# mmsyan/GoPairingBasedCryptography

Measured on AMD Instinct MI355X. Metric: BN254 pairings/s at batch 2^20 per GPU (+ G1/G2 scalar-mults/s at the same batch in roofline.scalar_mul), higher is better.
Workload: dtype int64; 1 GPU; configs[1]: batch of 1048576 independent bn254.Pair on random (G1,G2) points per GPU; batch_per_gpu=1048576

## Files before the change

gopairingbasedcryptography_amd/csrc/curve29.hip.hpp:

```cpp
#ifndef GPBC_CURVE29_HIP_HPP
#define GPBC_CURVE29_HIP_HPP
#include "tower29.hip.hpp"

namespace gpbc {

GPBC_INLINE Fe g_add(const Fe &a, const Fe &b) { return fe_add(a, b); }
GPBC_INLINE Fe g_sub(const Fe &a, const Fe &b) { return fe_sub(a, b); }
GPBC_INLINE Fe g_dbl(const Fe &a) { return fe_dbl(a); }
GPBC_INLINE Fe g_norm(const Fe &a) { return fe_norm(a); }
GPBC_INLINE Fe g_mul8n(const Fe &a) { return fe_mul8_norm(a); }
GPBC_INLINE Fe g_mul(const Fe &a, const Fe &b) { return fe_mul(a, b); }
GPBC_INLINE Fe g_sqr(const Fe &a) { return fe_sqr(a); }
GPBC_INLINE Fe g_inv(const Fe &a) { return fe_inv(a); }
GPBC_INLINE bool g_is_zero(const Fe &a) { return fe_is_zero(a); }
GPBC_INLINE void g_set_one(Fe &a) { a = fe_one(); }
GPBC_INLINE void g_set_zero(Fe &a) { a = fe_zero(); }
GPBC_INLINE F2 g_add(const F2 &a, const F2 &b) { return f2_add(a, b); }
GPBC_INLINE F2 g_sub(const F2 &a, const F2 &b) { return f2_sub(a, b); }
GPBC_INLINE F2 g_dbl(const F2 &a) { return f2_dbl(a); }
GPBC_INLINE F2 g_norm(const F2 &a) { return f2_norm(a); }
GPBC_INLINE F2 g_mul8n(const F2 &a) { return f2_mul8_norm(a); }
GPBC_INLINE F2 g_mul(const F2 &a, const F2 &b) { return f2_mul(a, b); }
GPBC_INLINE F2 g_sqr(const F2 &a) { return f2_sqr(a); }
GPBC_INLINE F2 g_inv(const F2 &a) { return f2_inv(a); }
// ... 48 lines not shown
    F Z1Z1 = g_sqr(p.z), Z2Z2 = g_sqr(q.z);
    F U1 = g_mul(p.x, Z2Z2), U2 = g_mul(q.x, Z1Z1);
    F S1 = g_mul(g_mul(p.y, q.z), Z2Z2), S2 = g_mul(g_mul(q.y, p.z), Z1Z1);
    F H = g_sub(U2, U1);
    F rr = g_sub(S2, S1);
    if (g_is_zero(H)) {
        if (g_is_zero(rr)) { jac_dbl(r, p); return; }
        jac_set_inf(r);
        return;
    }
    rr = g_norm(g_dbl(rr));
    F HH = g_sqr(H);
    F I = g_norm(g_dbl(g_dbl(HH)));
    F J = g_mul(H, I);
    F V = g_mul(U1, I);
    F x3 = g_norm(g_sub(g_sub(g_sqr(rr), J), g_dbl(V)));
    F y3 = g_norm(g_sub(g_mul(rr, g_sub(V, x3)), g_dbl(g_mul(S1, J))));
    F z3 = g_mul(g_norm(g_sub(g_sub(g_sqr(g_norm(g_add(p.z, q.z))), Z1Z1), Z2Z2)), H);
    r.x = x3; r.y = y3; r.z = z3; r.inf = false;
}
template <class F> GPBC_INLINE void jac_to_affine(AffP<F> &r, const JacP<F> &p) {
    if (p.inf) { g_set_zero(r.x); g_set_zero(r.y); r.inf = true; return; }
    F zi = g_inv(p.z);
    F zi2 = g_sqr(zi);
    r.x = g_mul(p.x, zi2);
    r.y = g_mul(p.y, g_mul(zi2, zi));
    r.inf = false;
}

struct GlvSplit { uint32_t k1[5], k2[5]; bool neg1, neg2; };

template <int NA, int NB, int NO> GPBC_INLINE void mp_mul(uint32_t (&out)[NO], const uint32_t (&a)[NA], const uint32_t (&b)[NB]) {
    uint64_t carry = 0;
#pragma unroll
    for (int k = 0; k < NO; k++) {
        uint64_t lo = carry, hi = 0;
#pragma unroll
        for (int i = 0; i < NA; i++) {
            const int j = k - i;
            if (j < 0 || j >= NB) continue;
            uint64_t p = (uint64_t)a[i] * (uint64_t)b[j];
            lo += p & 0xffffffffu;
            hi += p >> 32;
        }
        out[k] = (uint32_t)lo;
        carry = (lo >> 32) + hi;
    }
}
template <int N> GPBC_INLINE void mp_sub(uint32_t (&r)[N], const uint32_t (&a)[N], const uint32_t (&b)[N]) {
    uint64_t borrow = 0;
#pragma unroll
    for (int i = 0; i < N; i++) {
        uint64_t d = (uint64_t)a[i] - b[i] - borrow;
        r[i] = (uint32_t)d;
        borrow = (d >> 32) & 1;
    }
}
GPBC_INLINE void glv_split(GlvSplit &o, const uint32_t kin[8]) {
    constexpr uint32_t R32[8] = GLV_R32, G1[3] = GLV_G1, G2[5] = GLV_G2, A1[2] = GLV_A1, A2[4] = GLV_A2, B1[4] = GLV_B1ABS, B2[2] = GLV_B2;
    uint32_t k[8];
#pragma unroll
    for (int i = 0; i < 8; i++) k[i] = kin[i];
    for (int rep = 0; rep < 6; rep++) {
        uint32_t d[8];
        uint64_t borrow = 0;
#pragma unroll
        for (int i = 0; i < 8; i++) { uint64_t t = (uint64_t)k[i] - R32[i] - borrow; d[i] = (uint32_t)t; borrow = (t >> 32) & 1; }
#pragma unroll
        for (int i = 0; i < 8; i++) k[i] = borrow ? k[i] : d[i];
    }
    uint32_t p1[11], p2[13];
    mp_mul<8, 3, 11>(p1, k, G1);
    mp_mul<8, 5, 13>(p2, k, G2);
    uint32_t c1[3] = {p1[8], p1[9], p1[10]}, c2[5] = {p2[8], p2[9], p2[10], p2[11], p2[12]};
    uint32_t t1[5], t2[5], t3[5], t4[5], k5[5] = {k[0], k[1], k[2], k[3], k[4]}, r1[5], r2[5];
    mp_mul<3, 2, 5>(t1, c1, A1);
    mp_mul<5, 4, 5>(t2, c2, A2);
    mp_sub<5>(r1, k5, t1);
    mp_sub<5>(r1, r1, t2);
    mp_mul<3, 4, 5>(t3, c1, B1);
    mp_mul<5, 2, 5>(t4, c2, B2);
    mp_sub<5>(r2, t3, t4);
    o.neg1 = (r1[4] >> 31) != 0;
    o.neg2 = (r2[4] >> 31) != 0;
    uint32_t zero[5] = {0, 0, 0, 0, 0}, n1[5], n2[5];
    mp_sub<5>(n1, zero, r1);
    mp_sub<5>(n2, zero, r2);
#pragma unroll
    for (int i = 0; i < 5; i++) { o.k1[i] = o.neg1 ? n1[i] : r1[i]; o.k2[i] = o.neg2 ? n2[i] : r2[i]; }
}

GPBC_INLINE Fe glv_phi_x(const Fe &x) { constexpr int32_t B[NL] = GLV_BETA_G1; return fe_mul(x, fe_const(B)); }
GPBC_INLINE F2 glv_phi_x(const F2 &x) { constexpr int32_t B[NL] = GLV_BETA_G2; return f2_mul_fe(x, fe_const(B)); }
GPBC_INLINE Fe g_neg(const Fe &a) { return fe_neg(a); }
GPBC_INLINE F2 g_neg(const F2 &a) { return f2_neg(a); }

template <class F> GPBC_INLINE F g_sel(bool c, const F &a, const F &b);
template <> GPBC_INLINE Fe g_sel<Fe>(bool c, const Fe &a, const Fe &b) {
    Fe r;
#pragma unroll
    for (int i = 0; i < NL; i++) r.v[i] = c ? a.v[i] : b.v[i];
#ifdef GPBC_BOUNDS
    for (int i = 0; i < NL; i++) { r.lo[i] = a.lo[i] < b.lo[i] ? a.lo[i] : b.lo[i]; r.hi[i] = a.hi[i] > b.hi[i] ? a.hi[i] : b.hi[i]; }
    r.vb = a.vb > b.vb ? a.vb : b.vb;
#endif
    return r;
}
template <> GPBC_INLINE F2 g_sel<F2>(bool c, const F2 &a, const F2 &b) { return F2{g_sel<Fe>(c, a.a0, b.a0), g_sel<Fe>(c, a.a1, b.a1)}; }

template <class F> GPBC_INLINE JacP<F> jac_phi(const JacP<F> &p, bool flip) {
    return JacP<F>{glv_phi_x(p.x), flip ? g_neg(p.y) : p.y, p.z, p.inf};
}
struct alignas(16) TabQuad { int32_t a, b, c, d; };
template <class F> struct TabLayout;
template <> struct TabLayout<Fe> { static constexpr int ENTRY_DWORDS = 32; };
template <> struct TabLayout<F2> { static constexpr int ENTRY_DWORDS = 64; };
template <class F> constexpr int glv_table_dwords() { return 16 * TabLayout<F>::ENTRY_DWORDS; }
GPBC_INLINE void tab_put(TabQuad *q, const Fe &x, const Fe &y) {
    q[0] = TabQuad{x.v[0], x.v[1], x.v[2], x.v[3]};
    q[1] = TabQuad{x.v[4], x.v[5], x.v[6], x.v[7]};
    q[2] = TabQuad{x.v[8], y.v[0], y.v[1], y.v[2]};
    q[3] = TabQuad{y.v[3], y.v[4], y.v[5], y.v[6]};
    q[4] = TabQuad{y.v[7], y.v[8], 0, 0};
}
GPBC_INLINE void tab_get(const TabQuad *q, Fe &x, Fe &y) {
    TabQuad t0 = q[0], t1 = q[1], t2 = q[2], t3 = q[3], t4 = q[4];
    x.v[0] = t0.a; x.v[1] = t0.b; x.v[2] = t0.c; x.v[3] = t0.d; x.v[4] = t1.a; x.v[5] = t1.b; x.v[6] = t1.c; x.v[7] = t1.d; x.v[8] = t2.a;
    y.v[0] = t2.b; y.v[1] = t2.c; y.v[2] = t2.d; y.v[3] = t3.a; y.v[4] = t3.b; y.v[5] = t3.c; y.v[6] = t3.d; y.v[7] = t4.a; y.v[8] = t4.b;
    GPBC_B(set_class_n(x, 1.5); set_class_n(y, 1.5);)
}
GPBC_INLINE void tab_store(int32_t *mem, int idx, const AffP<Fe> &p) { tab_put(reinterpret_cast<TabQuad *>(mem + idx * 32), p.x, p.y); }
GPBC_INLINE void tab_store(int32_t *mem, int idx, const AffP<F2> &p) {
    TabQuad *q = reinterpret_cast<TabQuad *>(mem + idx * 64);
    tab_put(q, p.x.a0, p.x.a1);
    tab_put(q + 5, p.y.a0, p.y.a1);
}
GPBC_INLINE void tab_load(const int32_t *mem, int idx, AffP<Fe> &p) { tab_get(reinterpret_cast<const TabQuad *>(mem + idx * 32), p.x, p.y); p.inf = false; }
GPBC_INLINE void tab_load(const int32_t *mem, int idx, AffP<F2> &p) {
    const TabQuad *q = reinterpret_cast<const TabQuad *>(mem + idx * 64);
    tab_get(q, p.x.a0, p.x.a1);
    tab_get(q + 5, p.y.a0, p.y.a1);
    p.inf = false;
}
template <class F> GPBC_NOINLINE void glv_table29(int32_t *tab, F &W, const AffP<F> &p1, const AffP<F> &p2, bool flip) {
    F one;
    g_set_one(one);
    JacP<F> J[11];
    JacP<F> p1j{p1.x, p1.y, one, false};
    jac_dbl(J[0], p1j);
    jac_add_mixed(J[1], J[0], p1);
    jac_add_mixed(J[2], p1j, p2);
    jac_dbl(J[3], J[2]);
    jac_add(J[4], J[3], J[2]);
    JacP<F> d2 = jac_phi(J[0], flip), t2 = jac_phi(J[1], flip);
    jac_add_mixed(J[5], d2, p1);
    jac_add_mixed(J[6], J[0], p2);
    jac_add_mixed(J[7], t2, p1);
    jac_add_mixed(J[8], J[1], p2);
    jac_add_mixed(J[9], J[7], p1);
    jac_add_mixed(J[10], J[8], p2);
    F pre[11], l[11];
    F run = one;
    for (int i = 0; i < 11; i++) { pre[i] = run; run = g_mul(run, J[i].z); }
    W = run;
    run = one;
    for (int i = 10; i >= 0; i--) { l[i] = g_mul(pre[i], run); run = g_mul(run, J[i].z); }
    static constexpr int IDX[11] = {8, 12, 5, 10, 15, 6, 9, 7, 13, 11, 14};
    F l2d = one, l3d = one, l2t = one, l3t = one;
    for (int i = 0; i < 11; i++) {
        F l2 = g_sqr(l[i]), l3 = g_mul(l2, l[i]);
        tab_store(tab, IDX[i], AffP<F>{g_mul(J[i].x, l2), g_mul(J[i].y, l3), false});
        if (i == 0) { l2d = l2; l3d = l3; }
        if (i == 1) { l2t = l2; l3t = l3; }
    }
    tab_store(tab, 2, AffP<F>{g_mul(d2.x, l2d), g_mul(d2.y, l3d), false});
    tab_store(tab, 3, AffP<F>{g_mul(t2.x, l2t), g_mul(t2.y, l3t), false});
    F w2 = g_sqr(W), w3 = g_mul(w2, W);
    tab_store(tab, 4, AffP<F>{g_mul(p1.x, w2), g_mul(p1.y, w3), false});
    tab_store(tab, 1, AffP<F>{g_mul(p2.x, w2), g_mul(p2.y, w3), false});
}
template <class F> GPBC_INLINE void scalar_mul29_jac(JacP<F> &acc, const AffP<F> &base, const uint32_t k[8], int32_t *tab) {
    GlvSplit s;
    glv_split(s, k);
    jac_set_inf(acc);
    int top = 159;
    while (top >= 0 && !(((s.k1[top >> 5] | s.k2[top >> 5]) >> (top & 31)) & 1)) top--;
    if (base.inf || top < 0) return;
    AffP<F> p1{base.x, s.neg1 ? g_neg(base.y) : base.y, false};
    AffP<F> p2{glv_phi_x(base.x), s.neg2 ? g_neg(base.y) : base.y, false};
    F W;
    glv_table29<F>(tab, W, p1, p2, s.neg1 != s.neg2);
    for (int i = top >> 1; i >= 0; i--) {
        const int b = 2 * i;
        const int idx = 4 * (int)((s.k1[b >> 5] >> (b & 31)) & 3) + (int)((s.k2[b >> 5] >> (b & 31)) & 3);
        AffP<F> t;
        tab_load(tab, idx, t);
        jac_dbl(acc, acc);
        jac_dbl(acc, acc);
        if (idx) jac_add_mixed(acc, acc, t);
    }
    if (!acc.inf) acc.z = g_mul(acc.z, W);
}
struct GlsSplit { uint32_t k[4][3]; bool neg[4]; };
GPBC_INLINE void gls_split(GlsSplit &o, const uint32_t kin[8]) {
    constexpr uint32_t R32[8] = GLV_R32, G[4][7] = GLS_G, BM[4][4][3] = GLS_BMAG;
    constexpr int GN[4] = GLS_GNEG, BN[4][4] = GLS_BNEG;
    uint32_t k[8];
#pragma unroll
    for (int i = 0; i < 8; i++) k[i] = kin[i];
    for (int rep = 0; rep < 6; rep++) {
        uint32_t d[8];
        uint64_t borrow = 0;
#pragma unroll
        for (int i = 0; i < 8; i++) { uint64_t t = (uint64_t)k[i] - R32[i] - borrow; d[i] = (uint32_t)t; borrow = (t >> 32) & 1; }
#pragma unroll
        for (int i = 0; i < 8; i++) k[i] = borrow ? k[i] : d[i];
    }
    uint32_t c[4][3];
#pragma unroll
    for (int j = 0; j < 4; j++) {
        uint32_t p[11];
        mp_mul<8, 7, 11>(p, k, G[j]);
        c[j][0] = p[8]; c[j][1] = p[9]; c[j][2] = p[10];
    }
#pragma unroll
    for (int i = 0; i < 4; i++) {
        uint32_t acc[3] = {i == 0 ? k[0] : 0u, i == 0 ? k[1] : 0u, i == 0 ? k[2] : 0u};
#pragma unroll
        for (int j = 0; j < 4; j++) {
            uint32_t t[3], r[3];
            mp_mul<3, 3, 3>(t, c[j], BM[j][i]);
            const bool plus = (GN[j] != 0) != (BN[j][i] != 0);
            if (plus) {
                uint64_t cy = 0;
#pragma unroll
                for (int w = 0; w < 3; w++) { uint64_t v = (uint64_t)acc[w] + t[w] + cy; r[w] = (uint32_t)v; cy = v >> 32; }
            } else mp_sub<3>(r, acc, t);
            acc[0] = r[0]; acc[1] = r[1]; acc[2] = r[2];
        }
        o.neg[i] = (acc[2] >> 31) != 0;
        if (o.neg[i]) {
            uint32_t z[3] = {0, 0, 0}, r[3];
            mp_sub<3>(r, z, acc);
            acc[0] = r[0]; acc[1] = r[1]; acc[2] = r[2];
        }
        o.k[i][0] = acc[0]; o.k[i][1] = acc[1]; o.k[i][2] = acc[2];
    }
}
GPBC_NOINLINE void gls_table29(int32_t *tab, F2 &W, const AffP<F2> (&P)[4]) {
    F2 one = f2_one();
    static constexpr int IDX[11] = {3, 5, 6, 7, 9, 10, 11, 12, 13, 14, 15};
    JacP<F2> J[11];
    auto single = [&](int i) { return JacP<F2>{P[i].x, P[i].y, one, false}; };
    jac_add_mixed(J[0], single(0), P[1]);
    jac_add_mixed(J[1], single(0), P[2]);
    jac_add_mixed(J[2], single(1), P[2]);
    jac_add_mixed(J[3], J[0], P[2]);
    jac_add_mixed(J[4], single(0), P[3]);
    jac_add_mixed(J[5], single(1), P[3]);
    jac_add_mixed(J[6], J[0], P[3]);
    jac_add_mixed(J[7], single(2), P[3]);
    jac_add_mixed(J[8], J[1], P[3]);
    jac_add_mixed(J[9], J[2], P[3]);
    jac_add_mixed(J[10], J[3], P[3]);
    F2 pre[11], l[11];
    F2 run = one;
    for (int i = 0; i < 11; i++) { pre[i] = run; run = f2_mul(run, J[i].z); }
    W = run;
    run = one;
    for (int i = 10; i >= 0; i--) { l[i] = f2_mul(pre[i], run); run = f2_mul(run, J[i].z); }
    for (int i = 0; i < 11; i++) {
        F2 l2 = f2_sqr(l[i]), l3 = f2_mul(l2, l[i]);
        tab_store(tab, IDX[i], AffP<F2>{f2_mul(J[i].x, l2), f2_mul(J[i].y, l3), false});
    }
    F2 w2 = f2_sqr(W), w3 = f2_mul(w2, W);
    for (int i = 0; i < 4; i++) tab_store(tab, 1 << i, AffP<F2>{f2_mul(P[i].x, w2), f2_mul(P[i].y, w3), false});
}
GPBC_INLINE void scalar_mul29_gls(JacP<F2> &acc, const AffP<F2> &base, const uint32_t k[8], int32_t *tab) {
    GlsSplit s;
    gls_split(s, k);
    jac_set_inf(acc);
    int top = 95;
    while (top >= 0 && !(((s.k[0][top >> 5] | s.k[1][top >> 5] | s.k[2][top >> 5] | s.k[3][top >> 5]) >> (top & 31)) & 1)) top--;
    if (base.inf || top < 0) return;
    AffP<F2> P[4];
    P[0] = AffP<F2>{base.x, s.neg[0] ? f2_neg(base.y) : base.y, false};
    for (int i = 1; i < 4; i++) {
        const bool cj = i & 1;
        F2 y = f2_mul(cj ? f2_conj(base.y) : base.y, gamma29(i, 3));
        P[i] = AffP<F2>{f2_mul(cj ? f2_conj(base.x) : base.x, gamma29(i, 2)), s.neg[i] ? f2_neg(y) : y, false};
    }
    F2 W;
    gls_table29(tab, W, P);
    for (int i = top; i >= 0; i--) {
        const int w = i >> 5, b = i & 31;
        const int idx = (int)((s.k[0][w] >> b) & 1) | (int)(((s.k[1][w] >> b) & 1) << 1) | (int)(((s.k[2][w] >> b) & 1) << 2) | (int)(((s.k[3][w] >> b) & 1) << 3);
        AffP<F2> t;
        tab_load(tab, idx, t);
        jac_dbl(acc, acc);
        if (idx) jac_add_mixed(acc, acc, t);
    }
    if (!acc.inf) acc.z = f2_mul(acc.z, W);
}
GPBC_INLINE void scalar_mul29_best(JacP<Fe> &acc, const AffP<Fe> &base, const uint32_t k[8], int32_t *tab) { scalar_mul29_jac<Fe>(acc, base, k, tab); }
GPBC_INLINE void scalar_mul29_best(JacP<F2> &acc, const AffP<F2> &base, const uint32_t k[8], int32_t *tab) { scalar_mul29_gls(acc, base, k, tab); }

template <class F> GPBC_INLINE void scalar_mul29(AffP<F> &out, const AffP<F> &base, const uint32_t k[8], int32_t *tab) {
    JacP<F> acc;
    scalar_mul29_jac(acc, base, k, tab);
    jac_to_affine(out, acc);
}

template <class F, int K> GPBC_INLINE void jac_to_affine_batch(AffP<F> (&out)[K], const JacP<F> (&p)[K]) {
    F one, pre[K];
    g_set_one(one);
    F run = one;
    for (int j = 0; j < K; j++) {
        pre[j] = run;
        run = g_mul(run, p[j].inf ? one : p[j].z);
    }
    F inv = g_inv(run);
    for (int j = K - 1; j >= 0; j--) {
        F zi = g_mul(inv, pre[j]);
        inv = g_mul(inv, p[j].inf ? one : p[j].z);
        if (p[j].inf) { g_set_zero(out[j].x); g_set_zero(out[j].y); out[j].inf = true; continue; }
        F zi2 = g_sqr(zi);
        out[j].x = g_mul(p[j].x, zi2);
        out[j].y = g_mul(p[j].y, g_mul(zi2, zi));
        out[j].inf = false;
    }
}

}
#endif
```

gopairingbasedcryptography_amd/csrc/gpbc_curve.hip:

```cpp
#include "gpbc_common.hpp"
#include "curve29_oct.hip.hpp"
#include "fbindex29.hip.hpp"
#include "../../include/gpbc_bn254_indexed.h"

constexpr int SMUL_K = 1;
GPBC_KERNEL_G1 k_g1_scalar_mul(const uint8_t *__restrict__ bases, int shared_base, const uint8_t *__restrict__ scalars, uint8_t *__restrict__ out, size_t n, int32_t *__restrict__ tabws) {
    size_t t = (size_t)blockIdx.x * BLOCK + threadIdx.x;
    size_t T = (n + SMUL_K - 1) / SMUL_K;
    if (t >= T) return;
    JacP<Fe> res[SMUL_K];
    for (int j = 0; j < SMUL_K; j++) {
        size_t i = t + (size_t)j * T;
        if (i >= n) { jac_set_inf(res[j]); continue; }
        AffP<Fe> b = g1_load_aff(bases + (shared_base ? 0 : i * GPBC_G1_BYTES));
        uint32_t k[8];
        load_scalar(k, scalars + i * GPBC_SCALAR_BYTES);
        scalar_mul29_jac<Fe>(res[j], b, k, tabws + t * (size_t)glv_table_dwords<Fe>());
    }
    AffP<Fe> aff[SMUL_K];
    jac_to_affine_batch<Fe, SMUL_K>(aff, res);
    for (int j = 0; j < SMUL_K; j++) {
        size_t i = t + (size_t)j * T;
        if (i < n) g1_store_aff(out + i * GPBC_G1_BYTES, aff[j]);
    }
}
GPBC_KERNEL k_g2_scalar_mul(const uint8_t *__restrict__ bases, int shared_base, const uint8_t *__restrict__ scalars, uint8_t *__restrict__ out, size_t n, int32_t *__restrict__ tabws) {
    size_t t = (size_t)blockIdx.x * BLOCK + threadIdx.x;
    size_t T = (n + SMUL_K - 1) / SMUL_K;
    if (t >= T) return;
    JacP<F2> res[SMUL_K];
    for (int j = 0; j < SMUL_K; j++) {
        size_t i = t + (size_t)j * T;
        if (i >= n) { jac_set_inf(res[j]); continue; }
        AffP<F2> b = g2_load_aff(bases + (shared_base ? 0 : i * GPBC_G2_BYTES));
        uint32_t k[8];
        load_scalar(k, scalars + i * GPBC_SCALAR_BYTES);
        scalar_mul29_best(res[j], b, k, tabws + t * (size_t)glv_table_dwords<F2>());
    }
    AffP<F2> aff[SMUL_K];
    jac_to_affine_batch<F2, SMUL_K>(aff, res);
    for (int j = 0; j < SMUL_K; j++) {
        size_t i = t + (size_t)j * T;
        if (i < n) g2_store_aff(out + i * GPBC_G2_BYTES, aff[j]);
    }
}

constexpr size_t SMUL_QUAD_MAX = 16384;
GPBC_KERNEL_G1 k_g1_scalar_mul_quad(const uint8_t *__restrict__ bases, int shared_base, const uint8_t *__restrict__ scalars, uint8_t *__restrict__ out, size_t n, int32_t *__restrict__ tabws) {
    const size_t lane = (size_t)blockIdx.x * BLOCK + threadIdx.x, i = lane >> 2;
    const int q = (int)(lane & 3);
    if (i >= n) return;
    AffP<Fe> b = g1_load_aff(bases + (shared_base ? 0 : i * GPBC_G1_BYTES));
    uint32_t k[8];
    load_scalar(k, scalars + i * GPBC_SCALAR_BYTES);
    JacP<Fe> res;
    scalar_mul29_jac_quad<Fe>(res, b, k, tabws + i * (size_t)glv_table_dwords<Fe>(), q);
    AffP<Fe> aff;
    jac_to_affine(aff, res);
    if (q == 0) g1_store_aff(out + i * GPBC_G1_BYTES, aff);
}
GPBC_KERNEL k_g2_scalar_mul_quad(const uint8_t *__restrict__ bases, int shared_base, const uint8_t *__restrict__ scalars, uint8_t *__restrict__ out, size_t n, int32_t *__restrict__ tabws) {
    const size_t lane = (size_t)blockIdx.x * BLOCK + threadIdx.x, i = lane >> 2;
    const int q = (int)(lane & 3);
    if (i >= n) return;
    AffP<F2> b = g2_load_aff(bases + (shared_base ? 0 : i * GPBC_G2_BYTES));
    uint32_t k[8];
    load_scalar(k, scalars + i * GPBC_SCALAR_BYTES);
    JacP<F2> res;
    scalar_mul29_gls_quad(res, b, k, tabws + i * (size_t)glv_table_dwords<F2>(), q);
    AffP<F2> aff;
    jac_to_affine(aff, res);
    if (q == 0) g2_store_aff(out + i * GPBC_G2_BYTES, aff);
}

constexpr size_t SMUL_OCT_MAX = 2048;
GPBC_KERNEL k_g2_scalar_mul_oct(const uint8_t *__restrict__ bases, int shared_base, const uint8_t *__restrict__ scalars, uint8_t *__restrict__ out, size_t n, int32_t *__restrict__ tabws) {
    const size_t lane = (size_t)blockIdx.x * BLOCK + threadIdx.x, i = lane >> 3;
    const int q = (int)(lane & 7);
    if (i >= n) return;
    AffP<F2> b = g2_load_aff(bases + (shared_base ? 0 : i * GPBC_G2_BYTES));
    uint32_t k[8];
    load_scalar(k, scalars + i * GPBC_SCALAR_BYTES);
    JacP<F2> res;
    scalar_mul29_gls_oct(res, b, k, tabws + i * (size_t)glv_table_dwords<F2>(), q);
    AffP<F2> aff;
    jac_to_affine(aff, res);
    if (q == 0) g2_store_aff(out + i * GPBC_G2_BYTES, aff);
}

GPBC_KERNEL_G1 k_g1_sum_level(const uint8_t *__restrict__ in, size_t n_in, uint8_t *__restrict__ out, size_t n_out) {
    size_t t = (size_t)blockIdx.x * BLOCK + threadIdx.x;
    if (t >= n_out) return;
    JacP<Fe> acc;
    jac_set_inf(acc);
    for (size_t i = t; i < n_in; i += n_out) jac_add_mixed(acc, acc, g1_load_aff(in + i * GPBC_G1_BYTES));
    AffP<Fe> r;
    jac_to_affine(r, acc);
    g1_store_aff(out + t * GPBC_G1_BYTES, r);
}
GPBC_KERNEL k_g2_sum_level(const uint8_t *__restrict__ in, size_t n_in, uint8_t *__restrict__ out, size_t n_out) {
    size_t t = (size_t)blockIdx.x * BLOCK + threadIdx.x;
    if (t >= n_out) return;
    JacP<F2> acc;
    jac_set_inf(acc);
    for (size_t i = t; i < n_in; i += n_out) jac_add_mixed(acc, acc, g2_load_aff(in + i * GPBC_G2_BYTES));
    AffP<F2> r;
    jac_to_affine(r, acc);
    g2_store_aff(out + t * GPBC_G2_BYTES, r);
}

constexpr int FB_WINDOWS = 32, FB_DIGITS = 255, FB_ENTRIES = FB_WINDOWS * FB_DIGITS;
template <class F> __device__ __forceinline__ void fb_build_lane(const uint8_t *bases, size_t nbase, int32_t *table, uint8_t *base_inf, int32_t *tabws, size_t first, size_t count) {
    size_t t = (size_t)blockIdx.x * BLOCK + threadIdx.x;
    if (t >= count) return;
    const size_t e = first + t, b = e / FB_ENTRIES;
    const int rem = (int)(e % FB_ENTRIES), w = rem / FB_DIGITS, d = rem % FB_DIGITS + 1;
    constexpr size_t PT = sizeof(F) == sizeof(Fe) ? GPBC_G1_BYTES : GPBC_G2_BYTES;
    const uint8_t *bp = bases + b * PT;
    AffP<F> base;
    if constexpr (sizeof(F) == sizeof(Fe)) base = g1_load_aff(bp); else base = g2_load_aff(bp);
    if (rem == 0) base_inf[b] = base.inf ? 1 : 0;
    uint32_t k[8] = {0, 0, 0, 0, 0, 0, 0, 0};
    k[w >> 2] = (uint32_t)d << (8 * (w & 3));
    JacP<F> r;
    scalar_mul29_best(r, base, k, tabws + t * (size_t)glv_table_dwords<F>());
    AffP<F> a;
    jac_to_affine(a, r);
    tab_store(table + e * (size_t)TabLayout<F>::ENTRY_DWORDS, 0, a);
}
GPBC_KERNEL_G1 k_g1_fb_build(const uint8_t *__restrict__ bases, size_t nbase, int32_t *__restrict__ table, uint8_t *__restrict__ base_inf, int32_t *__restrict__ tabws, size_t first, size_t count) {
    fb_build_lane<Fe>(bases, nbase, table, base_inf, tabws, first, count);
}
GPBC_KERNEL k_g2_fb_build(const uint8_t *__restrict__ bases, size_t nbase, int32_t *__restrict__ table, uint8_t *__restrict__ base_inf, int32_t *__restrict__ tabws, size_t first, size_t count) {
    fb_build_lane<F2>(bases, nbase, table, base_inf, tabws, first, count);
}
template <class F, bool QUAD = false> __device__ __forceinline__ void fb_msm_lane(const int32_t *table, const uint8_t *base_inf, size_t nbase, const uint8_t *scalars,
                                                               size_t n_msm, size_t C, size_t n_chunks, uint8_t *partial) {
    const size_t lane = (size_t)blockIdx.x * BLOCK + threadIdx.x;
    size_t t = QUAD ? lane >> 2 : lane;
    const int q = (int)(lane & 3);
    if (t >= n_msm * n_chunks) return;
    const size_t m = t % n_msm, c = t / n_msm;
    JacP<F> acc;
    jac_set_inf(acc);
    const size_t j1 = (c + 1) * C < nbase ? (c + 1) * C : nbase;
    for (size_t j = c * C; j < j1; j++) {
        if (base_inf[j]) continue;
        uint32_t k[8];
        load_scalar(k, scalars + (m * nbase + j) * GPBC_SCALAR_BYTES);
        const int32_t *tb = table + j * (size_t)FB_ENTRIES * TabLayout<F>::ENTRY_DWORDS;
        for (int w = 0; w < FB_WINDOWS; w++) {
            const int d = (int)((k[w >> 2] >> (8 * (w & 3))) & 255u);
            if (d) {
                AffP<F> e;
                tab_load(tb + (size_t)(w * FB_DIGITS + d - 1) * TabLayout<F>::ENTRY_DWORDS, 0, e);
                if constexpr (QUAD) jac_add_mixed_quad(acc, e, q); else jac_add_mixed(acc, acc, e);
            }
        }
    }
    AffP<F> a;
    jac_to_affine(a, acc);
    if (QUAD && q != 0) return;
    if constexpr (sizeof(F) == sizeof(Fe)) g1_store_aff(partial + t * GPBC_G1_BYTES, a); else g2_store_aff(partial + t * GPBC_G2_BYTES, a);
}
GPBC_KERNEL_G1 k_g1_fb_msm(const int32_t *__restrict__ table, const uint8_t *__restrict__ base_inf, size_t nbase, const uint8_t *__restrict__ scalars,
                           size_t n_msm, size_t C, size_t n_chunks, uint8_t *__restrict__ partial) {
    fb_msm_lane<Fe>(table, base_inf, nbase, scalars, n_msm, C, n_chunks, partial);
}
GPBC_KERNEL k_g2_fb_msm(const int32_t *__restrict__ table, const uint8_t *__restrict__ base_inf, size_t nbase, const uint8_t *__restrict__ scalars,
                        size_t n_msm, size_t C, size_t n_chunks, uint8_t *__restrict__ partial) {
    fb_msm_lane<F2>(table, base_inf, nbase, scalars, n_msm, C, n_chunks, partial);
}

constexpr size_t FB_QUAD_MAX = 16384;
GPBC_KERNEL_G1 k_g1_fb_msm_quad(const int32_t *__restrict__ table, const uint8_t *__restrict__ base_inf, size_t nbase, const uint8_t *__restrict__ scalars,
                                size_t n_msm, size_t C, size_t n_chunks, uint8_t *__restrict__ partial) {
    fb_msm_lane<Fe, true>(table, base_inf, nbase, scalars, n_msm, C, n_chunks, partial);
}
GPBC_KERNEL k_g2_fb_msm_quad(const int32_t *__restrict__ table, const uint8_t *__restrict__ base_inf, size_t nbase, const uint8_t *__restrict__ scalars,
                             size_t n_msm, size_t C, size_t n_chunks, uint8_t *__restrict__ partial) {
    fb_msm_lane<F2, true>(table, base_inf, nbase, scalars, n_msm, C, n_chunks, partial);
}

static_assert(FBI_ENTRIES == FB_ENTRIES && FBI_WAVE == BLOCK && GPBC_INDEX_NONE == FBI_NONE, "fbindex29.hip.hpp restates the table geometry");
#ifndef GPBC_FBINDEX_GROUP_MIN
#define GPBC_FBINDEX_GROUP_MIN 64
#endif
template <class F> __device__ __forceinline__ void fb_indexed_kernel(const int32_t *table, const uint8_t *base_inf, size_t nbase, const uint32_t *index, FbIndexMap map, uint32_t terms,
                                                                     const uint8_t *scalars, uint8_t *out, uint8_t *ok_out) {
    const size_t i = fb_index_output(map, blockIdx.x, threadIdx.x);
    if (i >= map.n) return;
    constexpr size_t PT = sizeof(F) == sizeof(Fe) ? GPBC_G1_BYTES : GPBC_G2_BYTES;
    fb_indexed_lane<F>(table, base_inf, nbase, index + (i % map.P) * terms, terms, scalars + i * terms * GPBC_SCALAR_BYTES, out + i * PT, ok_out ? ok_out + i : nullptr,
                       [](uint32_t *k, const uint8_t *p) { load_scalar(k, p); },
                       [](uint8_t *p, const AffP<F> &a) { if constexpr (sizeof(F) == sizeof(Fe)) g1_store_aff(p, a); else g2_store_aff(p, a); });
}
GPBC_KERNEL_G1 k_g1_fb_indexed(const int32_t *__restrict__ table, const uint8_t *__restrict__ base_inf, size_t nbase, const uint32_t *__restrict__ index, FbIndexMap map, uint32_t terms,
                               const uint8_t *__restrict__ scalars, uint8_t *__restrict__ out, uint8_t *__restrict__ ok_out) {
    fb_indexed_kernel<Fe>(table, base_inf, nbase, index, map, terms, scalars, out, ok_out);
}
GPBC_KERNEL k_g2_fb_indexed(const int32_t *__restrict__ table, const uint8_t *__restrict__ base_inf, size_t nbase, const uint32_t *__restrict__ index, FbIndexMap map, uint32_t terms,
                            const uint8_t *__restrict__ scalars, uint8_t *__restrict__ out, uint8_t *__restrict__ ok_out) {
    fb_indexed_kernel<F2>(table, base_inf, nbase, index, map, terms, scalars, out, ok_out);
}

int point_sum_strided_dev(bool g2, const void *d_in, size_t n_in, void *d_out, size_t n_out, hipStream_t st) {
    if (g2) return GPBC_LAUNCH(k_g2_sum_level, grid_for(n_out), BLOCK, st, (const uint8_t *)d_in, n_in, (uint8_t *)d_out, n_out);
    return GPBC_LAUNCH(k_g1_sum_level, grid_for(n_out), BLOCK, st, (const uint8_t *)d_in, n_in, (uint8_t *)d_out, n_out);
}

extern "C" {

constexpr size_t FB_AUTO_MIN = 16384;
static int shared_base_mul_dev(bool g2, const void *d_base, const void *d_scalars, size_t n, void *d_out, hipStream_t st) {
    const size_t row_dwords = g2 ? (size_t)TabLayout<F2>::ENTRY_DWORDS : (size_t)TabLayout<Fe>::ENTRY_DWORDS;
    const size_t table_bytes = (size_t)FB_ENTRIES * row_dwords * sizeof(int32_t);
    Scratch tmp;
    if (tmp.open(st, 0, Scratch::padded(table_bytes) + 256) != GPBC_OK) return GPBC_ERR_WORKSPACE;
    int32_t *table = tmp.take<int32_t>(table_bytes);
    uint8_t *base_inf = tmp.take(256);
    const size_t tab_bytes = sizeof(int32_t) * (g2 ? (size_t)glv_table_dwords<F2>() : (size_t)glv_table_dwords<Fe>());
    int rc;
    {
        std::lock_guard<std::mutex> seq(g_ws_seq_mu);
        int32_t *tabws = nullptr;
        rc = stream_workspace(st, (size_t)FB_ENTRIES * tab_bytes, &tabws);
        if (rc == GPBC_OK) {
            if (g2) rc = GPBC_LAUNCH(k_g2_fb_build, grid_for(FB_ENTRIES), BLOCK, st, (const uint8_t *)d_base, 1, table, base_inf, tabws, 0, FB_ENTRIES);
            else rc = GPBC_LAUNCH(k_g1_fb_build, grid_for(FB_ENTRIES), BLOCK, st, (const uint8_t *)d_base, 1, table, base_inf, tabws, 0, FB_ENTRIES);
        }
    }
    if (rc == GPBC_OK) {
        if (g2) rc = GPBC_LAUNCH(k_g2_fb_msm, grid_for(n), BLOCK, st, table, base_inf, 1, (const uint8_t *)d_scalars, n, 1, 1, (uint8_t *)d_out);
        else rc = GPBC_LAUNCH(k_g1_fb_msm, grid_for(n), BLOCK, st, table, base_inf, 1, (const uint8_t *)d_scalars, n, 1, 1, (uint8_t *)d_out);
    }
    return rc;
}
static int scalar_mul_dev(bool g2, const void *d_bases, size_t nbase, const void *d_scalars, size_t n, void *d_out, void *stream) {
    if (!n) return GPBC_OK;
    if (!d_bases || !d_scalars || !d_out) return fail(GPBC_ERR_INVALID_ARG, "null pointer");
    if (nbase != 1 && nbase != n) return fail(GPBC_ERR_INVALID_ARG, "nbase must be 1 or n");
    TRY(bind_device());
    static_assert(SMUL_K == 1, "the table workspace is laid out for one point per lane");
    if (nbase == 1 && n >= FB_AUTO_MIN) {
        int rc = shared_base_mul_dev(g2, d_bases, d_scalars, n, d_out, (hipStream_t)stream);
        if (rc != GPBC_ERR_WORKSPACE) return rc;
    }
    const int shared = (nbase == 1 && n != 1) ? 1 : 0;
    const size_t pt = g2 ? GPBC_G2_BYTES : GPBC_G1_BYTES;
    const size_t tab_bytes = sizeof(int32_t) * (g2 ? (size_t)glv_table_dwords<F2>() : (size_t)glv_table_dwords<Fe>());
    hipStream_t st = (hipStream_t)stream;
    const size_t chunk = n < SMUL_CHUNK ? n : SMUL_CHUNK;
    std::lock_guard<std::mutex> seq(g_ws_seq_mu);
    int32_t *tabws = nullptr;
    TRY(stream_workspace(st, chunk * tab_bytes, &tabws));
    for (size_t off = 0; off < n; off += chunk) {
        const size_t m = n - off < chunk ? n - off : chunk;
        const uint8_t *b = (const uint8_t *)d_bases + (shared ? 0 : off * pt), *k = (const uint8_t *)d_scalars + off * GPBC_SCALAR_BYTES;
        uint8_t *o = (uint8_t *)d_out + off * pt;
        if (g2 && n <= SMUL_OCT_MAX) TRY(GPBC_LAUNCH(k_g2_scalar_mul_oct, grid_for(8 * m), BLOCK, st, b, shared, k, o, m, tabws));
        else if (g2 && n <= SMUL_QUAD_MAX) TRY(GPBC_LAUNCH(k_g2_scalar_mul_quad, grid_for(4 * m), BLOCK, st, b, shared, k, o, m, tabws));
        else if (n <= SMUL_QUAD_MAX) TRY(GPBC_LAUNCH(k_g1_scalar_mul_quad, grid_for(4 * m), BLOCK, st, b, shared, k, o, m, tabws));
        else if (g2) TRY(GPBC_LAUNCH(k_g2_scalar_mul, grid_for(m), BLOCK, st, b, shared, k, o, m, tabws));
        else TRY(GPBC_LAUNCH(k_g1_scalar_mul, grid_for(m), BLOCK, st, b, shared, k, o, m, tabws));
    }
    return GPBC_OK;
}
int gpbc_g1_scalar_mul_batch_dev(const void *b, size_t nb, const void *s, size_t n, void *o, void *st) { return scalar_mul_dev(false, b, nb, s, n, o, st); }
int gpbc_g2_scalar_mul_batch_dev(const void *b, size_t nb, const void *s, size_t n, void *o, void *st) { return scalar_mul_dev(true, b, nb, s, n, o, st); }

constexpr size_t SUM_FANIN = 32;
size_t gpbc_sum_workspace_bytes(size_t n, int is_g2) {
    size_t pt = is_g2 ? GPBC_G2_BYTES : GPBC_G1_BYTES, total = 0;
    while (n > 1) { n = (n + SUM_FANIN - 1) / SUM_FANIN; total += n * pt; }
    return total + pt;
}
static int sum_dev(bool g2, const void *d_pts, size_t n, void *d_out, void *d_ws, size_t ws_bytes, void *stream) {
    if (!d_out) return fail(GPBC_ERR_INVALID_ARG, "null pointer");
    TRY(bind_device());
    size_t pt = g2 ? GPBC_G2_BYTES : GPBC_G1_BYTES;
    if (!n) { HIP_TRY(hipMemsetAsync(d_out, 0, pt, (hipStream_t)stream)); return GPBC_OK; }
    if (!d_pts || !d_ws) return fail(GPBC_ERR_INVALID_ARG, "null pointer");
    if (ws_bytes < gpbc_sum_workspace_bytes(n, g2)) return fail(GPBC_ERR_WORKSPACE, "workspace too small");
    const uint8_t *in = (const uint8_t *)d_pts;
    uint8_t *ws = (uint8_t *)d_ws;
    size_t n_in = n;
    for (;;) {
        size_t n_out = (n_in + SUM_FANIN - 1) / SUM_FANIN;
        uint8_t *out = n_out == 1 ? (uint8_t *)d_out : ws;
        if (g2) TRY(GPBC_LAUNCH(k_g2_sum_level, grid_for(n_out), BLOCK, (hipStream_t)stream, in, n_in, out, n_out));
        else TRY(GPBC_LAUNCH(k_g1_sum_level, grid_for(n_out), BLOCK, (hipStream_t)stream, in, n_in, out, n_out));
        if (n_out == 1) break;
        in = out; ws += n_out * pt; n_in = n_out;
    }
    return GPBC_OK;
}
int gpbc_g1_sum_dev(const void *p, size_t n, void *o, void *w, size_t wb, void *s) { return sum_dev(false, p, n, o, w, wb, s); }
int gpbc_g2_sum_dev(const void *p, size_t n, void *o, void *w, size_t wb, void *s) { return sum_dev(true, p, n, o, w, wb, s); }

constexpr size_t SMUL_PIPE_CHUNK = 131072;
static int small_mul_run(SmallKind kind, CallLane &lane, SmallCall *const *calls, size_t nc) {
    const bool g2 = kind == CALL_G2_MUL;
    const size_t tab_bytes = sizeof(int32_t) * (g2 ? (size_t)glv_table_dwords<F2>() : (size_t)glv_table_dwords<Fe>());
    return small_rows_run(lane, calls, nc, [&](const uint8_t *const *in, const uint8_t *const *, uint8_t *const *out, size_t N) {
        TRY(lane.reserve(0, N * tab_bytes));
        if (g2) return GPBC_LAUNCH(k_g2_scalar_mul_oct, grid_for(8 * N), BLOCK, lane.stream, in[0], 0, in[1], out[0], N, (int32_t *)lane.dev);
        return GPBC_LAUNCH(k_g1_scalar_mul_quad, grid_for(4 * N), BLOCK, lane.stream, in[0], 0, in[1], out[0], N, (int32_t *)lane.dev);
    });
}
constexpr size_t SMUL_SHARD_MIN = 4096;
static int scalar_mul_host(bool g2, const void *bases, size_t nbase, const void *scalars, size_t n, void *out) {
    if (!n) return GPBC_OK;
    if (!bases || !scalars || !out) return fail(GPBC_ERR_INVALID_ARG, "null pointer");
    if (nbase != 1 && nbase != n) return fail(GPBC_ERR_INVALID_ARG, "nbase must be 1 or n");
    const size_t pt = g2 ? GPBC_G2_BYTES : GPBC_G1_BYTES;
    const bool shared = nbase == 1 && n != 1;
    return host_call_sharded(n, SMUL_SHARD_MIN, HostCall().input(bases, pt, shared).input(scalars, GPBC_SCALAR_BYTES).output(out, pt),
                             HostRoute{g2 ? CALL_G2_MUL : CALL_G1_MUL, small_mul_run, SMALL_CALL_MAX_UNITS, 0, shared ? 0 : SMUL_PIPE_CHUNK},
                             [=](const DevCols &d, size_t m, hipStream_t st) { return scalar_mul_dev(g2, d.in[0], shared ? 1 : m, d.in[1], m, d.out[0], st); });
}
// ... 269 lines not shown
```

Measured before the change: 7.513 million pairings/s.

## Use signed-window GLV scalar multiplication for G1 with co-Z odd-multiple table

Replaces the G1 scalar multiplication path with a GLV split plus width-5 signed odd-digit windows. A 16-entry table of odd multiples is built with co-Z additions and made affine with a shared inverse. Fewer additions per scalar bit are intended, with parity corrections at the end. The change only affects the G1 scalar-mult kernel, not the pairing metric headline.

```diff
diff --git a/gopairingbasedcryptography_amd/csrc/curve29.hip.hpp b/gopairingbasedcryptography_amd/csrc/curve29.hip.hpp
--- a/gopairingbasedcryptography_amd/csrc/curve29.hip.hpp
+++ b/gopairingbasedcryptography_amd/csrc/curve29.hip.hpp
@@ -374,7 +374,94 @@
     }
     if (!acc.inf) acc.z = f2_mul(acc.z, W);
 }
-GPBC_INLINE void scalar_mul29_best(JacP<Fe> &acc, const AffP<Fe> &base, const uint32_t k[8], int32_t *tab) { scalar_mul29_jac<Fe>(acc, base, k, tab); }
+constexpr int SW_W = 5, SW_ROWS = 1 << (SW_W - 1), SW_MASK = (1 << SW_W) - 1;
+static_assert(SW_ROWS == 16, "the per-lane table block holds 16 rows");
+constexpr int sw_windows(int top) { return top / SW_W + 1; }
+template <int N> GPBC_INLINE uint32_t sw_window(const uint32_t (&k)[N], int j, int n) {
+    const int p = SW_W * j + 1, wi = p >> 5, sh = p & 31;
+    uint32_t lo = 0, hi = 0;
+#pragma unroll
+    for (int i = 0; i < N; i++) { lo = wi == i ? k[i] : lo; hi = wi + 1 == i ? k[i] : hi; }
+    const uint32_t u = (uint32_t)((((uint64_t)hi << 32) | lo) >> sh) & (uint32_t)SW_MASK;
+    return j == n - 1 ? u | (uint32_t)SW_ROWS : u;
+}
+GPBC_INLINE int sw_digit(uint32_t u) { return 2 * (int)u - SW_MASK; }
+template <class F> GPBC_INLINE void sw_row(AffP<F> &t, const int32_t *tab, uint32_t u, bool neg) {
+    const bool pos = (u & (uint32_t)SW_ROWS) != 0;
+    tab_load(tab, (int)((pos ? u : ~u) & (uint32_t)(SW_ROWS - 1)), t);
+    t.y = g_sel<F>(neg == pos, g_neg(t.y), t.y);
+}
+template <class F> GPBC_INLINE JacP<F> jac_sel(bool c, const JacP<F> &a, const JacP<F> &b) {
+    return JacP<F>{g_sel<F>(c, a.x, b.x), g_sel<F>(c, a.y, b.y), g_sel<F>(c, a.z, b.z), c ? a.inf : b.inf};
+}
+template <class F> GPBC_NOINLINE void sw_table29(int32_t *tab, F &W, const AffP<F> &p) {
+    F one;
+    g_set_one(one);
+    F X[SW_ROWS], Y[SW_ROWS], h[SW_ROWS - 1];
+    F A = g_sqr(p.x), B = g_sqr(p.y);
+    F B4 = g_norm(g_dbl(g_dbl(B)));
+    X[0] = g_mul(p.x, B4);
+    Y[0] = g_mul(B, g_norm(g_dbl(B4)));
+    F E = g_norm(g_add(g_dbl(A), A));
+    F dx = g_norm(g_sub(g_sqr(E), g_dbl(X[0])));
+    F dy = g_norm(g_sub(g_mul(E, g_sub(X[0], dx)), Y[0]));
+    for (int i = 0; i + 1 < SW_ROWS; i++) {
+        h[i] = g_norm(g_sub(dx, X[i]));
+        F C = g_sqr(h[i]);
+        F W1 = g_mul(dx, C), W2 = g_mul(X[i], C);
+        F rr = g_norm(g_sub(dy, Y[i]));
+        F A1 = g_mul(dy, g_sub(W1, W2));
+        F x3 = g_norm(g_sub(g_sub(g_sqr(rr), W1), W2));
+        X[i + 1] = x3;
+        Y[i + 1] = g_norm(g_sub(g_mul(rr, g_norm(g_sub(W1, x3))), A1));
+        dx = W1; dy = A1;
+    }
+    tab_store(tab, SW_ROWS - 1, AffP<F>{g_mul(X[SW_ROWS - 1], one), g_mul(Y[SW_ROWS - 1], one), false});
+    F run = h[SW_ROWS - 2];
+    for (int i = SW_ROWS - 2; i >= 0; i--) {
+        if (i < SW_ROWS - 2) run = g_mul(run, h[i]);
+        F l2 = g_sqr(run), l3 = g_mul(l2, run);
+        tab_store(tab, i, AffP<F>{g_mul(X[i], l2), g_mul(Y[i], l3), false});
+    }
+    W = g_mul(g_norm(g_dbl(p.y)), run);
+}
+template <class F> GPBC_INLINE void scalar_mul29_sw(JacP<F> &acc, const AffP<F> &base, const uint32_t k[8], int32_t *tab) {
+    GlvSplit s;
+    glv_split(s, k);
+    jac_set_inf(acc);
+    int top = 159;
+    while (top >= 0 && !(((s.k1[top >> 5] | s.k2[top >> 5]) >> (top & 31)) & 1)) top--;
+    if (base.inf || top < 0) return;
+    F W;
+    sw_table29<F>(tab, W, base);
+    const int n = sw_windows(top);
+    AffP<F> t1, t2;
+    sw_row(t1, tab, sw_window(s.k1, n - 1, n), s.neg1);
+    sw_row(t2, tab, sw_window(s.k2, n - 1, n), s.neg2);
+    acc.x = t1.x; acc.y = t1.y; g_set_one(acc.z); acc.inf = false;
+    t2.x = glv_phi_x(t2.x);
+    jac_add_mixed(acc, acc, t2);
+    for (int j = n - 2; j >= 0; j--) {
+        sw_row(t1, tab, sw_window(s.k1, j, n), s.neg1);
+        sw_row(t2, tab, sw_window(s.k2, j, n), s.neg2);
+#pragma unroll 1
+        for (int d = 0; d < SW_W; d++) jac_dbl(acc, acc);
+        jac_add_mixed(acc, acc, t1);
+        t2.x = glv_phi_x(t2.x);
+        jac_add_mixed(acc, acc, t2);
+    }
+    AffP<F> q, q1, q2;
+    tab_load(tab, 0, q);
+    q1 = AffP<F>{q.x, g_sel<F>(s.neg1, q.y, g_neg(q.y)), false};
+    q2 = AffP<F>{glv_phi_x(q.x), g_sel<F>(s.neg2, q.y, g_neg(q.y)), false};
+    JacP<F> r;
+    jac_add_mixed(r, acc, q1);
+    acc = jac_sel<F>(!(s.k1[0] & 1), r, acc);
+    jac_add_mixed(r, acc, q2);
+    acc = jac_sel<F>(!(s.k2[0] & 1), r, acc);
+    if (!acc.inf) acc.z = g_mul(acc.z, W);
+}
+GPBC_INLINE void scalar_mul29_best(JacP<Fe> &acc, const AffP<Fe> &base, const uint32_t k[8], int32_t *tab) { scalar_mul29_sw<Fe>(acc, base, k, tab); }
 GPBC_INLINE void scalar_mul29_best(JacP<F2> &acc, const AffP<F2> &base, const uint32_t k[8], int32_t *tab) { scalar_mul29_gls(acc, base, k, tab); }
 
 template <class F> GPBC_INLINE void scalar_mul29(AffP<F> &out, const AffP<F> &base, const uint32_t k[8], int32_t *tab) {
diff --git a/gopairingbasedcryptography_amd/csrc/gpbc_curve.hip b/gopairingbasedcryptography_amd/csrc/gpbc_curve.hip
--- a/gopairingbasedcryptography_amd/csrc/gpbc_curve.hip
+++ b/gopairingbasedcryptography_amd/csrc/gpbc_curve.hip
@@ -15,7 +15,7 @@
         AffP<Fe> b = g1_load_aff(bases + (shared_base ? 0 : i * GPBC_G1_BYTES));
         uint32_t k[8];
         load_scalar(k, scalars + i * GPBC_SCALAR_BYTES);
-        scalar_mul29_jac<Fe>(res[j], b, k, tabws + t * (size_t)glv_table_dwords<Fe>());
+        scalar_mul29_best(res[j], b, k, tabws + t * (size_t)glv_table_dwords<Fe>());
     }
     AffP<Fe> aff[SMUL_K];
     jac_to_affine_batch<Fe, SMUL_K>(aff, res);
```

Measured after the change: 7.495 million pairings/s. Within noise of the previous version (-0.2%).
